# second-state/qwen3_asr_rs

Hardware: AMD Instinct MI355X
Metric: audio-seconds/sec (RTFx) Qwen3-ASR-0.6B greedy, 30s clips (higher is better)
Workload: dtype bf16; 1 GPU; Qwen3-ASR-0.6b bf16, batch=1 x 30s synthetic 16kHz clip per GPU, 100 new tokens (fixed, EOS ignored); clips_per_gpu=1, parallelism=dp1 (independent utterances per GPU, no data-path collective)

## Files before the change

### qwen3_asr_rs_amd/csrc/engine.cpp

```cpp
#include <hip/hip_runtime.h>

#include <sched.h>

#include <chrono>
#include <cmath>
#include <cstdio>
#include <cstring>
#include <map>
#include <memory>
#include <mutex>
#include <thread>

#include "engine_internal.h"

using namespace q3a;

namespace {

thread_local std::string g_last_error;

constexpr int kGemvMaxSeq = 2;

template <typename T>
void upload(DevBuf& b, const std::vector<T>& v, hipStream_t s) {
// ... 416 lines not shown
  }
  void enqueue_beam_round() {
    const int W = beam_w_, S = B, U = B / W;
    BeamTopkArgs t{};
    t.logits = logits.as<float>(); t.S = S; t.V = d.vocab; t.W = W;
    t.cand_val = beam_cand_val.as<float>(); t.cand_idx = beam_cand_idx.as<int>();
    t.part_max = beam_part_max.as<float>(); t.part_sum = beam_part_sum.as<float>();
    t.out_ids = beam_topk_ids.as<int>(); t.out_lp = beam_topk_lp.as<float>();
    timed(Q3A_KC_ARGMAX, 0, [&] { KCHK(launch_beam_topk(t, stream)); });
    BeamAdvanceArgs a{};
    a.U = U; a.W = W; a.topk_ids = t.out_ids; a.topk_lp = t.out_lp;
    a.score = beam_score.as<float>(); a.finished = beam_finished.as<uint8_t>();
    a.parent = beam_parent.as<int>(); a.token = beam_token.as<int>(); a.feed = beam_feed.as<int>();
    a.hist_parent = beam_hist_parent.as<int>(); a.hist_token = beam_hist_token.as<int>(); a.hist_lp = beam_hist_lp.as<float>();
    a.hist_cap = max_new; a.state = beam_state.as<int>();
    a.pos = d_pos.as<int>(); a.lo = beam_lo.as<int>(); a.hi_bias = -1;
    a.host_progress = host_prog_dev + 2; a.eos0 = kEos0; a.eos1 = kEos1;
    timed(Q3A_KC_ARGMAX, 0, [&] { KCHK(launch_beam_advance(a, stream)); });
    KvReorderArgs r{};
    r.kcache = kcache.p; r.vcache = vcache.p; r.elem_bytes = (int)kv_elem(); r.layers = d.dec_layers; r.S = S; r.n_kv = d.n_kv; r.max_ctx = max_ctx;
    r.parent = a.parent; r.lo = a.lo; r.hi = a.pos; r.hi_bias = -1; r.all_done = a.state + BEAM_ST_ALL_DONE;
    timed(Q3A_KC_OTHER, 0, [&] { KCHK(launch_kv_reorder(r, stream)); });
    timed(Q3A_KC_OTHER, 0, [&] { enqueue_set_tokens(a.feed); });
  }
};

enum class Stage { None, Batch, Mel, Encoded, Decoding };

class CallState {
  Stage stage_ = Stage::None;
  int beam_w_ = 0;
  bool fixed_mode_ = false;
  bool head_logits_ = true;
 public:
  bool at(Stage s) const { return stage_ >= s; }
  const int& beam_w() const { return beam_w_; }
  bool fixed_mode() const { return fixed_mode_; }
  const bool& head_logits() const { return head_logits_; }
  void advance(Stage s) { if (stage_ < s) stage_ = s; }
  void rewind(Stage s) {
    if (stage_ > s) stage_ = s;
    if (stage_ < Stage::Decoding) end_search();
  }
  void drop_decode_state() { rewind(Stage::Encoded); }
  void require(Stage s, const char* text) const { if (stage_ < s) fail(text); }
  void require(Stage s, const std::string& text) const { require(s, text.c_str()); }
  void begin_search(int W) { beam_w_ = W; }
  void end_search() { beam_w_ = 0; }
  void begin_call(bool fixed, bool keep_logits) { fixed_mode_ = fixed; head_logits_ = keep_logits; }
  void begin_step_call() { head_logits_ = true; }
};

}

struct q3a_engine : CallState {
  Dims d;
  ArenaLayout L;
  q3a_opts opts{};
  int device = 0;
  hipStream_t stream = nullptr;
  uint8_t* arena = nullptr;
  bool own_arena = false;
  uint32_t arena_flags = 0;
  std::string err;

  DevBuf dft, filt_t, pos_emb;
  int rope_positions = 0;

  int B = 0;
  std::vector<int64_t> n_samples, pcm_off, mel_off;
  std::vector<int> n_frames, n_chunks, T, tok_off;
  int total_chunks = 0, total_T = 0, max_frames = 0;
  std::vector<int> P, seq_off;
  int total_P = 0, max_ctx = 0, max_new = 0;
  std::vector<AttnSeg> enc_segs_h;
  int enc_max_seg = 0;

  DevBuf pcm, d_pcm_off, d_n_samples, d_mel_off, d_n_frames, mel, gmax, d_chunk_utt, d_chunk_frame0;
  DevBuf conv1, conv2, conv3, conv3_rowmap, convout_rowmap;
  DevBuf enc_x, enc_ln, enc_qkv, enc_ctx, enc_ffn, enc_segs, audio_embeds;
  DevBuf ids, audio_rowmap, row_seq, row_pos, dec_segs, last_rows;
  DevBuf dec_x, dec_ln, dec_qkv, dec_ctx, dec_act;
  DevBuf lm_q_buf, lm_qs_buf;
  const int8_t* lm_q = nullptr; const float* lm_qs = nullptr;
  int lm_q_cols = 0;
  DevBuf enc_ctx16, dec_ctx16;
  DevBuf dec_q16;
  int n_cu = 256;
  int* host_prog = nullptr;
  int* host_prog_dev = nullptr;
  DevBuf zero_page;
  int part_stride = 0, attn_nsplit = 0;
  size_t kv_layer_elems = 0;

  int gsize = 32;
  int k_parallel_groups = 1, k_skinny_q = 1, k_dattn_batched_min_wgs = 128, k_skinny_glu_hp3 = 1, k_lm_head_prune = 1;
  std::vector<hipStream_t> chain_streams;
  std::vector<hipEvent_t> join_ev;
  hipEvent_t fork_ev = nullptr;

  static constexpr size_t kGraphCacheMax = 16;
  std::vector<std::pair<std::string, hipGraphExec_t>> graph_cache;
  int pos_hi_ = 0, live_nsplit_ = 0;
  int min_P_ = 0;

  hipStream_t up_stream = nullptr;
  void* pin_p = nullptr;
  size_t pin_cap = 0;
  std::vector<hipEvent_t> up_ev;
  hipEvent_t up_t0 = nullptr, up_t1 = nullptr;
  q3a_io_timings io{};
  bool geom_valid = false;

  q3a_timings timings{};
  hipEvent_t ev[5] = {nullptr, nullptr, nullptr, nullptr, nullptr};
  std::vector<ProfEvent>* prof = nullptr;
  Taps taps;

  bool logit_bias_on_ = false;
  int logit_bias_finite_ = 0;
  bool sampling_on_ = false;
  uint32_t samp_words_[4] = {0, 0, 0, 0};
  bool logit_bias_eos_open_ = true;
  bool repetition_on_ = false;
  float rep_penalty_ = 1.f;
  int rep_ngram_ = 0;

  DecodeStep step{StepView{d, L, opts, arena, arena_flags, stream, chain_streams, join_ev, fork_ev, n_cu, host_prog_dev, prof, taps, lm_q, lm_qs, lm_q_cols,
                           B, max_ctx, max_new, gsize, live_nsplit_, attn_nsplit, min_P_, part_stride, beam_w(), kv_layer_elems, head_logits(),
                           k_parallel_groups, k_skinny_q, k_dattn_batched_min_wgs, k_skinny_glu_hp3, k_lm_head_prune, logit_bias_on_, sampling_on_, repetition_on_}};

  bool precise() const { return step.precise(); }
  bool token_lp() const { return step.token_lp(); }
  bool kv_f32() const { return step.kv_f32(); }
  size_t kv_elem() const { return step.kv_elem(); }
  size_t act_elem() const { return precise() ? 4 : 2; }
  bool valu_attn() const { return precise() || opts.valu_attention; }
  const float* wf(uint64_t off) const { return step.wf(off); }
  const uint16_t* wh(uint64_t off) const { return step.wh(off); }

  void tap(const char* name, const void* ptr, size_t bytes) { step.tap(name, ptr, bytes); }
  void tap_act(const char* name, const void* ptr, size_t elems) {
    if (!opts.debug_taps || elems == 0 || opts.debug_taps == 2) return;
    if (precise()) return tap(name, ptr, elems * 4);
    KCHK(launch_from_bf16((const uint16_t*)ptr, taps.reserve(name, elems * 4).as<float>(), elems, stream));
  }

  void act_gemm(const DevBuf& x, int lda, const uint16_t* W, int M, int N, int K, const GemmEpilogue& ep, bool glu) {
    if (precise()) KCHK(launch_gemm(x.as<float>(), lda, W, M, N, K, ep, glu, true, stream));
    else KCHK(launch_gemm16(x.as<uint16_t>(), lda, W, M, N, K, ep, glu, stream));
// ... 149 lines not shown
    upload(d_n_frames, n_frames, stream);
    upload(d_chunk_utt, chunk_utt, stream);
    upload(d_chunk_frame0, chunk_frame0, stream);
    upload(convout_rowmap, convout_map, stream);
    upload(conv3_rowmap, conv3_map, stream);
    upload(enc_segs, enc_segs_h, stream);
    mel.ensure((size_t)mo * 4);
    gmax.ensure((size_t)b * 4);
    HIPCHK(hipStreamSynchronize(stream));
    B = b;
    geom_valid = true;
    advance(Stage::Batch);
  }

  void upload_pcm(const float* host, const int64_t* ns, int b) {
    set_batch(ns, b);
    int64_t src = 0;
    for (int u = 0; u < b; ++u) {
      HIPCHK(hipMemcpyAsync(pcm.as<float>() + pcm_off[u], host + src, (size_t)ns[u] * 4, hipMemcpyHostToDevice, stream));
      src += ns[u];
    }
    HIPCHK(hipStreamSynchronize(stream));
  }

  void upload_ptrs_and_mel(const float* const* ptrs, const int64_t* ns, int b) {
    const auto w0 = std::chrono::steady_clock::now();
    set_batch(ns, b);
    static const int mode = [] { const char* e = getenv("Q3A_UPLOAD_MODE"); return e ? atoi(e) : 1; }();
    static const int thr_env = [] { const char* e = getenv("Q3A_UPLOAD_THREADS"); return e ? atoi(e) : -1; }();
    static const int pieces_env = [] { const char* e = getenv("Q3A_UPLOAD_PIECES"); return e ? atoi(e) : 8; }();
    io = q3a_io_timings{};
    io.mode = mode;
    HIPCHK(hipEventRecord(ev[0], stream));
    const size_t total = (size_t)(pcm_off[b - 1] + ((ns[b - 1] + 3) & ~int64_t(3))) * 4;
    bool staged = mode != 0;
    if (staged && total > pin_cap) {
      if (up_stream) HIPCHK(hipStreamSynchronize(up_stream));
      if (pin_p) (void)hipHostFree(pin_p);
      pin_p = nullptr; pin_cap = 0;
      const size_t want = (total + (size_t(1) << 20) - 1) & ~((size_t(1) << 20) - 1);
      if (hipHostMalloc(&pin_p, want, hipHostMallocDefault) == hipSuccess && pin_p) pin_cap = want;
      else { (void)hipGetLastError(); pin_p = nullptr; staged = false; io.mode = 0; }
    }
    if (!staged) {
      for (int u = 0; u < b; ++u)
        HIPCHK(hipMemcpyAsync(pcm.as<float>() + pcm_off[u], ptrs[u], (size_t)ns[u] * 4, hipMemcpyHostToDevice, stream));
      HIPCHK(hipStreamSynchronize(stream));
      io.pieces = b;
      run_mel();
      HIPCHK(hipEventRecord(ev[1], stream));
      io.stage_ms = std::chrono::duration<float, std::milli>(std::chrono::steady_clock::now() - w0).count();
      return;
    }
    if (!up_stream) {
      HIPCHK(hipStreamCreateWithFlags(&up_stream, hipStreamNonBlocking));
      HIPCHK(hipEventCreate(&up_t0));
      HIPCHK(hipEventCreate(&up_t1));
    }
    HIPCHK(hipStreamSynchronize(up_stream));
    const int want_pieces = std::max(1, std::min(b, pieces_env));
    std::vector<int> first;
    {
      const size_t per = (total + want_pieces - 1) / want_pieces;
      size_t acc = 0;
      first.push_back(0);
      for (int u = 0; u < b; ++u) {
// ... 12 lines not shown
    io.pieces = np;
    io.threads = nthr;
    std::vector<std::atomic<int>> ready(np);
    for (auto& r : ready) r.store(0, std::memory_order_relaxed);
    std::atomic<int> next{0};
    uint8_t* const pin = (uint8_t*)pin_p;
    auto copy_piece = [&](int p) {
      for (int u = first[p]; u < first[p + 1]; ++u) memcpy(pin + (size_t)pcm_off[u] * 4, ptrs[u], (size_t)ns[u] * 4);
      ready[p].store(1, std::memory_order_release);
    };
    struct Joiner {
      std::vector<std::thread> th;
      ~Joiner() { for (auto& t : th) if (t.joinable()) t.join(); }
    } workers;
    for (int t = 0; t < nthr; ++t)
      workers.th.emplace_back([&] { for (int p; (p = next.fetch_add(1, std::memory_order_relaxed)) < np;) copy_piece(p); });
    MelBatch mb{pcm.as<float>(), d_pcm_off.as<int64_t>(), d_n_samples.as<int64_t>(), d_mel_off.as<int64_t>(),
                d_n_frames.as<int>(), mel.as<float>(), gmax.as<unsigned>()};
    HIPCHK(hipEventRecord(up_t0, up_stream));
    for (int p = 0; p < np; ++p) {
      if (nthr == 0) copy_piece(p);
      for (unsigned spins = 0; !ready[p].load(std::memory_order_acquire);)
        if (++spins > 256) sched_yield();
      const int u0 = first[p], u1 = first[p + 1];
      const size_t o0 = (size_t)pcm_off[u0] * 4, o1 = (size_t)(pcm_off[u1 - 1] + ns[u1 - 1]) * 4;
      HIPCHK(hipMemcpyAsync((uint8_t*)pcm.p + o0, pin + o0, o1 - o0, hipMemcpyHostToDevice, up_stream));
      HIPCHK(hipEventRecord(up_ev[p], up_stream));
      HIPCHK(hipStreamWaitEvent(stream, up_ev[p], 0));
      MelBatch piece = mb;
      piece.pcm_off += u0; piece.n_samples += u0; piece.mel_off += u0; piece.n_frames += u0; piece.gmax_key += u0;
      int mf = 0;
      for (int u = u0; u < u1; ++u) mf = std::max(mf, n_frames[u]);
      KCHK(launch_mel(piece, u1 - u0, mf, dft.as<float>(), filt_t.as<float>(), stream));
    }
    HIPCHK(hipEventRecord(up_t1, up_stream));
    io.stage_ms = std::chrono::duration<float, std::milli>(std::chrono::steady_clock::now() - w0).count();
    mel_done();
    HIPCHK(hipEventRecord(ev[1], stream));
  }

  void run_mel() {
    MelBatch mb{pcm.as<float>(), d_pcm_off.as<int64_t>(), d_n_samples.as<int64_t>(), d_mel_off.as<int64_t>(),
                d_n_frames.as<int>(), mel.as<float>(), gmax.as<unsigned>()};
    KCHK(launch_mel(mb, B, max_frames, dft.as<float>(), filt_t.as<float>(), stream));
    mel_done();
  }
  void mel_done() {
    advance(Stage::Mel);
    size_t bytes = 0;
    for (int u = 0; u < B; ++u) bytes += (size_t)n_frames[u] * d.n_mels * 4;
    tap("mel", mel.p, bytes);
  }

  void run_encoder() {
    require(Stage::Mel, "q3a_encode: no mel (call q3a_mel first)");
    const int C = d.conv_ch, D = d.enc_d, Fn = d.enc_ffn;
    const int H1 = Dims::conv_len(d.n_mels), W1 = Dims::conv_len(d.chunk_frames());
    const int H2 = Dims::conv_len(H1), W2 = Dims::conv_len(W1);
    const int H3 = Dims::conv_len(H2), W3 = Dims::conv_len(W2);
    const bool sp = precise();
    const size_t nch = (size_t)total_chunks;
    const size_t ae = act_elem();
    conv1.ensure(nch * H1 * W1 * C * ae);
    conv2.ensure(nch * H2 * W2 * C * ae);
    conv3.ensure(nch * H3 * W3 * C * ae);
    const size_t Tt = (size_t)total_T;
    const bool qkv16 = !valu_attn();
    enc_x.ensure(Tt * D * 4); enc_ln.ensure(Tt * D * ae); enc_qkv.ensure(Tt * 3 * D * (qkv16 ? 2 : 4));
    enc_ctx.ensure(Tt * D * (valu_attn() ? 4 : ae));
    if (valu_attn() && !sp) enc_ctx16.ensure(Tt * D * 2);
    enc_ffn.ensure(Tt * Fn * ae); audio_embeds.ensure(Tt * d.enc_out * 4);

    ChunkTable ct{d_chunk_utt.as<int>(), d_chunk_frame0.as<int>()};
    KCHK(launch_conv1(mel.as<float>(), d_mel_off.as<int64_t>(), d_n_frames.as<int>(), ct, total_chunks, d.n_mels,
                      d.chunk_frames(), wf(L.conv1_w), wf(L.conv1_b), C, conv1.as<float>(), stream, act16(conv1)));
    tap_act("conv1", conv1.p, nch * H1 * W1 * C);
    {
// ... 50 lines not shown
      KCHK(launch_layernorm(enc_x.as<float>(), wf(e.ln2_w), wf(e.ln2_b), enc_ln.as<float>(), total_T, D, 1e-5f, stream, act16(enc_ln)));
      {
        GemmEpilogue ep; act_out(ep, enc_ffn); ep.ldo = Fn; ep.bias = wf(e.fc1_b); ep.act = 1;
        act_gemm(enc_ln, D, wh(e.fc1_w), total_T, Fn, D, ep, false);
      }
      {
        GemmEpilogue ep; ep.out = enc_x.as<float>(); ep.ldo = D; ep.bias = wf(e.fc2_b); ep.resid = enc_x.as<float>();
        act_gemm(enc_ffn, Fn, wh(e.fc2_w), total_T, D, Fn, ep, false);
      }
      if (li == 0) tap("enc_layer0", enc_x.p, Tt * D * 4);
      if (opts.debug_taps == 1 && knobs().layer_taps.load() != 0) {
        char name[32];
        snprintf(name, sizeof(name), "E%02d_x", li);
        tap(name, enc_x.p, Tt * D * 4);
      }
    }
    tap("enc_last", enc_x.p, Tt * D * 4);
    KCHK(launch_layernorm(enc_x.as<float>(), wf(L.ln_post_w), wf(L.ln_post_b), enc_ln.as<float>(), total_T, D, 1e-5f, stream, act16(enc_ln)));
    {
      GemmEpilogue ep; act_out(ep, enc_ffn); ep.ldo = D; ep.bias = wf(L.proj1_b); ep.act = 1;
      act_gemm(enc_ln, D, wh(L.proj1_w), total_T, D, D, ep, false);
    }
    {
      GemmEpilogue ep; ep.out = audio_embeds.as<float>(); ep.ldo = d.enc_out; ep.bias = wf(L.proj2_b);
      act_gemm(enc_ffn, D, wh(L.proj2_w), total_T, d.enc_out, D, ep, false);
    }
    tap("audio_embeds", audio_embeds.p, Tt * d.enc_out * 4);
    HIPCHK(hipGetLastError());
    advance(Stage::Encoded);
  }

  void setup_prompts(const int32_t* ids_h, const int32_t* lens, int b, int max_new_req, bool before_encoder = false) {
    if (!before_encoder) require_encoded("q3a_prefill", b);
    P.assign(lens, lens + b);
    end_search();
    seq_off.resize(b);
    std::vector<int> rowseq, rowpos, amap((size_t)total_T, -1), last(b);
    int off = 0, maxP = 0;
    for (int s = 0; s < b; ++s) {
      seq_off[s] = off;
      int na = 0;
      for (int i = 0; i < P[s]; ++i) {
        rowseq.push_back(s);
        rowpos.push_back(i);
        int id = ids_h[off + i];
        if (id < 0 || id >= d.vocab) fail("q3a_prefill: token id out of range");
        if (id == kAudioPad) {
          if (na >= T[s]) fail("q3a_prefill: more <|audio_pad|> tokens than encoder tokens");
          amap[(size_t)tok_off[s] + na] = off + i;
          ++na;
        }
      }
      if (na != T[s]) fail("q3a_prefill: number of <|audio_pad|> tokens does not match the encoder output length");
      if (P[s] <= 0) fail("q3a_prefill: empty prompt");
      last[s] = off + P[s] - 1;
      off += P[s];
      maxP = std::max(maxP, P[s]);
    }
    total_P = off;
    max_new = std::min(std::max(max_new_req, 1), opts.max_new_tokens);
    max_ctx = ((maxP + max_new + 1 + 127) / 128) * 128;
    pos_hi_ = maxP;
    min_P_ = *std::min_element(P.begin(), P.end());
    {
      static const int pad = [] { const char* e = getenv("Q3A_CTX_PAD"); return e ? atoi(e) : 0; }();
      if (pad > 0) max_ctx += (pad + 127) / 128 * 128;
    }
    ensure_rope(max_ctx + 1);
    std::vector<int> ids_v(ids_h, ids_h + total_P);
    std::vector<AttnSeg> segs(b);
    for (int s = 0; s < b; ++s)
      segs[s] = AttnSeg{seq_off[s], P[s], (int64_t)s * d.n_kv * max_ctx * 128};
    upload(ids, ids_v, stream);
    upload(row_seq, rowseq, stream);
    upload(row_pos, rowpos, stream);
    upload(audio_rowmap, amap, stream);
    upload(last_rows, last, stream);
    upload(dec_segs, segs, stream);
    upload(step.d_pos, P, stream);
    const size_t Pt = (size_t)total_P, H = d.hidden;
    dec_x.ensure(Pt * H * 4); dec_ln.ensure(Pt * H * act_elem()); dec_qkv.ensure(Pt * d.qkv_dim() * 4);
    dec_ctx.ensure(Pt * d.q_dim() * (valu_attn() ? 4 : act_elem())); dec_act.ensure(Pt * d.inter * act_elem());
    if (!valu_attn()) dec_q16.ensure(Pt * d.q_dim() * 2);
    if (valu_attn() && !precise()) dec_ctx16.ensure(Pt * d.q_dim() * 2);
    kv_layer_elems = (size_t)b * d.n_kv * max_ctx * 128;
    step.kcache.ensure(kv_layer_elems * d.dec_layers * kv_elem());
    step.vcache.ensure(kv_layer_elems * d.dec_layers * kv_elem());
    step.rope_cur.ensure((size_t)b * 128 * 4);
    {
      Knobs& kn = knobs();
      const int gs = kn.decode_group_size.load();
      gsize = (gs >= 1 && gs <= 32) ? gs : 32;
      k_parallel_groups = kn.decode_parallel_groups.load(); k_skinny_q = kn.skinny_q.load();
      k_dattn_batched_min_wgs = kn.dattn_batched_min_wgs.load();
      k_skinny_glu_hp3 = kn.skinny_glu_hp3.load();
      k_lm_head_prune = kn.lm_head_prune.load();
    }
    const size_t ng = (size_t)step.n_groups(b);
    step.nn_x.ensure(ng * 32 * H * 2); step.nn_ss.ensure((size_t)ng * (H / 8) * 32 * 4);
    step.x_dec.ensure((size_t)b * H * 4); step.next_tok.ensure((size_t)b * 4); step.forced_tok.ensure((size_t)b * 4); step.draft_accepted.ensure((size_t)b * 8);
    step.out_ids.ensure((size_t)b * max_new * 4); step.step_count.ensure((size_t)b * 4); step.done.ensure((size_t)b);
    step.s_ln.ensure((size_t)b * H * 4); step.s_qkv.ensure((size_t)b * d.qkv_dim() * 4); step.s_ctx.ensure(ng * 32 * d.q_dim() * 4);
    step.s_act.ensure(ng * 32 * d.inter * 4); step.logits.ensure((size_t)b * d.vocab * 4);
    part_stride = std::max(128, (d.vocab + 3) / 4);
    step.part_val.ensure((size_t)b * part_stride * 4); step.part_idx.ensure((size_t)b * part_stride * 4);
    if (token_lp()) { step.part_sum.ensure((size_t)b * part_stride * 4); step.out_lp.ensure((size_t)b * max_new * 4); }
    if (sampling_on_) { step.samp_max.ensure((size_t)b * sample_chunks(d.vocab) * 4); step.samp_sum.ensure((size_t)b * sample_chunks(d.vocab) * 4); }
    {
      const size_t nblk4 = ((size_t)(d.vocab + 15) / 16 + 3) & ~size_t(3);
      step.blk_lo.ensure(nblk4 * 4); step.blk_hi.ensure(nblk4 * 4);
    }
    attn_nsplit = (max_ctx + dattn_keys_per_split(kv_f32()) - 1) / dattn_keys_per_split(kv_f32());
    {
      const size_t n_stat = (size_t)b * d.n_q * attn_nsplit;
      step.attn_pm.ensure((n_stat + 8) * 4); step.attn_pl.ensure((n_stat + 8) * 4);
      step.attn_po.ensure(n_stat * 128 * 4);
      if (knobs().poison_attn_partials.load() != 0) {
        HIPCHK(hipMemsetAsync(step.attn_pm.p, 0xFF, step.attn_pm.cap, stream));
        HIPCHK(hipMemsetAsync(step.attn_pl.p, 0xFF, step.attn_pl.cap, stream));
        HIPCHK(hipMemsetAsync(step.attn_po.p, 0xFF, step.attn_po.cap, stream));
      }
    }
    HIPCHK(hipMemsetAsync(step.step_count.p, 0, (size_t)b * 4, stream));
    HIPCHK(hipMemsetAsync(step.done.p, 0, (size_t)b, stream));
    HIPCHK(hipMemsetAsync(step.n_done.p, 0, 64, stream));
    HIPCHK(hipMemsetAsync(step.out_ids.p, 0, (size_t)b * max_new * 4, stream));
    if (token_lp()) HIPCHK(hipMemsetAsync(step.out_lp.p, 0, (size_t)b * max_new * 4, stream));
    HIPCHK(hipStreamSynchronize(stream));
    for (auto cs : chain_streams) HIPCHK(hipStreamSynchronize(cs));
    __atomic_store_n(&host_prog[0], 0, __ATOMIC_RELAXED);
    __atomic_store_n(&host_prog[1], 0, __ATOMIC_RELAXED);
    drain_retired_graphs();
    {
      bool any = false;
      DecodeStep::each_buf(step, [&](DevBuf& sb) { any = any || sb.grew; sb.grew = false; });
      if (any) drop_graphs();
    }
  }

  void run_prefill() {
    run_prefill_layers();
    const int H = d.hidden;
    KCHK(launch_gather_rows(dec_x.as<float>(), last_rows.as<int>(), B, H, step.x_dec.as<float>(), stream));
    tap("dec_last_hidden", step.x_dec.p, (size_t)B * H * 4);
    step.run_head(0);
    tap("logits", step.logits.p, (size_t)B * d.vocab * 4);
    HIPCHK(hipGetLastError());
    advance(Stage::Decoding);
  }

  void run_prefill_layers() {
    drop_decode_state();
    const int H = d.hidden, I = d.inter, QD = d.q_dim(), QKV = d.qkv_dim();
    const bool sp = precise();
    KCHK(launch_embed(ids.as<int>(), total_P, wh(L.embed), H, kAudioPad, dec_x.as<float>(), stream));
    KCHK(launch_scatter_rows(audio_embeds.as<float>(), audio_rowmap.as<int>(), total_T, d.hidden, dec_x.as<float>(), stream));
    tap("dec_embed", dec_x.p, (size_t)total_P * H * 4);
    AttnArgs at{};
    at.q = dec_qkv.as<float>(); at.q_rs = QKV; at.kv_hs = (int64_t)max_ctx * 128; at.kv_rs = 128;
    at.o = dec_ctx.as<float>(); at.o_rs = QD; at.segs = dec_segs.as<AttnSeg>(); at.n_segs = B;
    at.max_len = *std::max_element(P.begin(), P.end()); at.n_kv_heads = d.n_kv;
    at.scale_div = sqrtf((float)d.head_dim);
    at.o16 = valu_attn() ? nullptr : dec_ctx.as<uint16_t>();
    if (!valu_attn()) { at.q16 = dec_q16.as<uint16_t>(); at.q_rs = QD; }
    const DevBuf& ctx_in = (valu_attn() && !sp) ? dec_ctx16 : dec_ctx;
    auto proj_gemm = [&](const DevBuf& x, const DecodeStep::Proj& p, GemmEpilogue ep) {
      ep.bias = p.bias;
      act_gemm(x, p.K, p.W, total_P, p.N, p.K, ep, p.mode == 2);
    };
    const bool fuse_rope = knobs().fuse_qkrope.load() != 0 && !valu_attn() && !precise() && d.head_dim == 128 && gemm256_eligible(total_P, QKV, H) && H % 64 == 0;
// ... 301 lines not shown
    return exec;
  }
  hipGraphExec_t graph_for_step() {
    const std::string sig = make_graph_sig();
    for (size_t i = 0; i < graph_cache.size(); ++i)
      if (graph_cache[i].first == sig) {
        if (i + 1 != graph_cache.size()) std::rotate(graph_cache.begin() + i, graph_cache.begin() + i + 1, graph_cache.end());
        return graph_cache.back().second;
      }
    const hipGraphExec_t exec = capture_graph([&] { enqueue_step(); });
    ++graph_captures_;
    if (graph_cache.size() >= kGraphCacheMax) {
      retired_graphs.push_back(graph_cache.front().second);
      graph_cache.erase(graph_cache.begin());
    }
    graph_cache.emplace_back(sig, exec);
    return exec;
  }
  std::vector<hipGraphExec_t> retired_graphs;
  int32_t graph_captures_ = 0;
  void drain_retired_graphs() {
    for (auto ge : retired_graphs) (void)hipGraphExecDestroy(ge);
    retired_graphs.clear();
  }
  void drop_graphs() {
    drain_retired_graphs();
    for (auto& ge : graph_cache) (void)hipGraphExecDestroy(ge.second);
    graph_cache.clear();
  }

  void decode_steps(int n) {
    require(Stage::Decoding, "decode: no prefill state");
    if (n <= 0) return;
    const bool eager = !opts.use_graph || prof;
    const int kps = dattn_keys_per_split(kv_f32());
    for (int i = 0; i < n; ++i) {
      live_nsplit_ = step.uses_key_splits() ? std::min(attn_nsplit, pos_hi_ / kps + 1) : attn_nsplit;
      if (eager) enqueue_step();
      else HIPCHK(hipGraphLaunch(graph_for_step(), stream));
      ++pos_hi_;
    }
    if (eager) HIPCHK(hipGetLastError());
  }

  int max_new_request(int max_new_req, int fixed_new) const { return fixed_new > 0 ? fixed_new : max_new_req > 0 ? max_new_req : opts.max_new_tokens; }
  std::pair<std::vector<int32_t>, std::vector<int32_t>> asr_prompts(const int32_t* lang_ids, int n_prefix) const {
    return concat_prompts(B, [&](int s, int32_t* dst) {
      int32_t len = 0;
      q3a_build_prompt(T[s], lang_ids, n_prefix, dst, &len);
      return len;
    });
  }

  template <class Prompts>
  void whole_path_front(const char* what, const float* const* pcm16k, const int64_t* ns_in, int n, int width, int max_new_req, Prompts&& prompts) {
    if (!pcm16k || !ns_in || n < 1) fail(std::string(what) + ": bad argument");
    require_utterance_ptrs(what, pcm16k, n);
    HIPCHK(hipSetDevice(device));
    const int b = n * width;
    std::vector<const float*> ptrs((size_t)b);
    std::vector<int64_t> ns((size_t)b);
    for (int s = 0; s < b; ++s) { ptrs[s] = pcm16k[s / width]; ns[s] = ns_in[s / width]; }
    set_batch(ns.data(), b);
    auto&& [ids_v, lens_v] = prompts();
    setup_prompts(ids_v.data(), lens_v.data(), b, max_new_req, true);
    timings = q3a_timings{};
    upload_ptrs_and_mel(ptrs.data(), ns.data(), b);
    run_encoder();
  }

  void run_resident(int fixed_new, bool front_done = false) {
    if (!front_done) {
      HIPCHK(hipEventRecord(ev[0], stream));
      run_mel();
      HIPCHK(hipEventRecord(ev[1], stream));
      run_encoder();
    }
    HIPCHK(hipEventRecord(ev[2], stream));
    run_prefill();
    HIPCHK(hipEventRecord(ev[3], stream));
    int steps = 0;
    static const bool host_timing = [] { const char* e = getenv("Q3A_DEBUG_HOST_TIMING"); return e && atoi(e) != 0; }();
    const auto h0 = std::chrono::steady_clock::now();
    if (fixed_new > 0) {
      steps = fixed_new - 1;
      decode_steps(steps);
      if (host_timing) fprintf(stderr, "[q3a host timing] %d graph launches enqueued in %.1f us\n", steps,
                               std::chrono::duration<double, std::micro>(std::chrono::steady_clock::now() - h0).count());
    } else {
      steps = run_ahead(host_prog, max_new - 1, "greedy");
    }
    HIPCHK(hipEventRecord(ev[4], stream));
    HIPCHK(hipStreamSynchronize(stream));
    HIPCHK(hipGetLastError());
    decode_timings(steps);
  }

  void fetch_ids(int32_t* out, int stride, int32_t* out_lens) {
    if (!at(Stage::Decoding) || beam_w() > 0) fail("q3a_fetch_ids: nothing generated");
    fetch_generated<int32_t>(nullptr, out, stride, out_lens);
  }
  void fetch_logprobs(float* out, int stride, int32_t* out_lens) {
    if (!token_lp()) fail("q3a_fetch_logprobs: the engine was created without opts.token_logprobs = 1");
    require(Stage::Decoding, "q3a_fetch_logprobs: nothing generated");
    fetch_generated<float>(&step.out_lp, out, stride, out_lens);
  }
  template <class T> void fetch_generated(const DevBuf* vals, T* out, int stride, int32_t* out_lens) {
    std::vector<int> ids((size_t)B * max_new);
    std::vector<T> v(vals ? ids.size() : 0);
    HIPCHK(hipMemcpy(ids.data(), step.out_ids.p, ids.size() * 4, hipMemcpyDeviceToHost));
    if (vals) HIPCHK(hipMemcpy(v.data(), vals->p, v.size() * sizeof(T), hipMemcpyDeviceToHost));
    generated_lens(ids, out_lens);
    for (int s = 0; s < B; ++s)
      for (int i = 0; i < std::min(out_lens[s], stride); ++i) out[(size_t)s * stride + i] = vals ? v[(size_t)s * max_new + i] : (T)ids[(size_t)s * max_new + i];
  }
  void generated_lens(const std::vector<int>& all, int32_t* out_lens) {
    std::vector<int> sc(B);
    HIPCHK(hipMemcpy(sc.data(), step.step_count.p, (size_t)B * 4, hipMemcpyDeviceToHost));
    for (int s = 0; s < B; ++s) {
      int n = std::min(sc[s], max_new), len = 0;
      for (; len < n; ++len) {
        int t = all[(size_t)s * max_new + len];
        if (!fixed_mode() && (t == kEos0 || t == kEos1)) break;
      }
      out_lens[s] = len;
    }
  }

  int beam_dbg_S_ = 0, beam_dbg_W_ = 0;
  int* beam_prog() const { return host_prog + 2; }

  void beam_check(const char* what, int W) const {
    if (W < 1 || W > BEAM_MAX_W) fail(std::string(what) + ": width must be 1..8");
    if (B % W != 0) fail(std::string(what) + ": the batch of " + std::to_string(B) + " sequences is not divisible by width " + std::to_string(W));
    if (B > 32) fail(std::string(what) + ": utterances x width = " + std::to_string(B) + " exceeds 32 sequences");
    for (int s = 0; s < B; ++s)
      if (P[s] != P[s / W * W]) fail(std::string(what) + ": the prompts of utterance " + std::to_string(s / W) + " differ in length (its " + std::to_string(W) + " slots must hold the same prompt)");
    if (d.vocab < W) fail(std::string(what) + ": vocabulary smaller than the width");
  }
  void set_logit_bias(const int32_t* ids, const float* bias, int n, float default_bias) {
    const char* what = "q3a_set_logit_bias";
    require_asr(what);
    const int V = d.vocab;
    if (n < 0 || (n > 0 && (!ids || !bias))) fail(std::string(what) + ": bad argument");
    if (!(default_bias == 0.f || default_bias == -INFINITY)) fail(std::string(what) + ": default_bias must be 0 or -inf");
    std::vector<float> b((size_t)V, default_bias);
    std::vector<uint8_t> seen((size_t)V, 0);
    for (int i = 0; i < n; ++i) {
      const int id = ids[i];
      if (id < 0 || id >= V) fail(std::string(what) + ": id " + std::to_string(id) + " is outside the vocabulary (" + std::to_string(V) + ")");
      if (seen[id]) fail(std::string(what) + ": duplicate id " + std::to_string(id));
// ... 139 lines not shown
      std::stable_sort(order.begin(), order.end(), [&](int x, int y) { return sc[u * W + x] > sc[u * W + y]; });
      for (int k = 0; k < W; ++k) {
        const int q = u * W + order[k];
        toks.clear(); lps.clear();
        for (int r = R - 1, cur = q; r >= 0; --r) {
          const size_t h = (size_t)r * S + cur;
          if (ht[h] >= 0) { toks.push_back(ht[h]); lps.push_back(hl[h]); }
          cur = hp[h];
        }
        std::reverse(toks.begin(), toks.end());
        std::reverse(lps.begin(), lps.end());
        const int n_lp = (int)toks.size();
        if (fin[q] && !toks.empty()) toks.pop_back();
        const int n = (int)toks.size();
        if (n > stride) fail("q3a_beam_fetch: a hypothesis has " + std::to_string(n) + " ids, more than stride " + std::to_string(stride));
        const size_t o = (size_t)u * W + k;
        for (int i = 0; i < n; ++i) out[o * stride + i] = toks[i];
        out_lens[o] = n;
        if (out_scores) out_scores[o] = sc[q];
        if (out_fin) out_fin[o] = fin[q];
        if (out_lp)
          for (int i = 0; i < n_lp && i < stride + 1; ++i) out_lp[o * (stride + 1) + i] = lps[i];
      }
    }
  }

  ~q3a_engine() {
    drop_graphs();
    for (auto cs : chain_streams) (void)hipStreamDestroy(cs);
    for (auto ce : join_ev) (void)hipEventDestroy(ce);
    if (fork_ev) (void)hipEventDestroy(fork_ev);
    if (own_arena && arena) (void)hipFree(arena);
    if (host_prog) (void)hipHostFree(host_prog);
    if (up_stream) { (void)hipStreamSynchronize(up_stream); (void)hipStreamDestroy(up_stream); }
    if (pin_p) (void)hipHostFree(pin_p);
    for (auto ue : up_ev) (void)hipEventDestroy(ue);
    if (up_t0) (void)hipEventDestroy(up_t0);
    if (up_t1) (void)hipEventDestroy(up_t1);
    for (auto& x : ev)
      if (x) (void)hipEventDestroy(x);
    if (stream) (void)hipStreamDestroy(stream);
  }
};


namespace q3a {
void set_thread_error(const std::string& msg) { g_last_error = msg; }
void set_error(q3a_engine* e, const char* msg) {
  if (e) e->err = msg;
  g_last_error = msg;
}
}

extern "C" {

void q3a_opts_default(q3a_opts* o) {
  memset(o, 0, sizeof(*o));
  o->precise = 0;
  o->max_new_tokens = 4096;
  o->use_graph = 1;
  o->debug_taps = 0;
}

static int32_t create_impl(const char* model_dir, int32_t device, void* dev_arena, uint64_t bytes, const q3a_opts* opts,
                           q3a_engine** out) {
  q3a_engine* e = nullptr;
// ... 331 lines not shown
  if (next_ids) HIPCHK(hipMemcpy(next_ids, e->step.next_tok.p, (size_t)B * 4, hipMemcpyDeviceToHost));
  Q3A_CATCH(e)
}

int32_t q3a_decode_step(q3a_engine* e, int32_t* next_ids, uint8_t* done, float* logits_out) {
  if (!e) return 1;
  Q3A_TRY(e)
  e->require_asr("q3a_decode_step");
  if (e->beam_w() > 0) fail("q3a_decode_step: a beam search owns the decode state (q3a_beam_step; a new q3a_prefill returns to the greedy step)");
  HIPCHK(hipSetDevice(e->device));
  {
    std::vector<int> pos(e->B);
    HIPCHK(hipMemcpy(pos.data(), e->step.d_pos.p, (size_t)e->B * 4, hipMemcpyDeviceToHost));
    for (int s = 0; s < e->B; ++s)
      if (pos[s] + 1 > e->max_ctx) fail("q3a_decode_step: KV cache capacity exhausted (max_new_tokens reached)");
  }
  e->begin_step_call();
  e->decode_steps(1);
  HIPCHK(hipStreamSynchronize(e->stream));
  HIPCHK(hipGetLastError());
  if (next_ids) HIPCHK(hipMemcpy(next_ids, e->step.next_tok.p, (size_t)e->B * 4, hipMemcpyDeviceToHost));
  if (done) HIPCHK(hipMemcpy(done, e->step.done.p, (size_t)e->B, hipMemcpyDeviceToHost));
  if (logits_out) HIPCHK(hipMemcpy(logits_out, e->step.logits.p, (size_t)e->B * e->d.vocab * 4, hipMemcpyDeviceToHost));
  Q3A_CATCH(e)
}

int32_t q3a_set_next_tokens(q3a_engine* e, const int32_t* ids, int32_t B) {
  if (!e) return 1;
  Q3A_TRY(e)
  HIPCHK(hipSetDevice(e->device));
  if (!e->at(Stage::Decoding) || B != e->B || e->beam_w() > 0) fail("q3a_set_next_tokens: no decode state / batch mismatch");
  for (int s = 0; s < B; ++s)
    if (ids[s] < 0 || ids[s] >= e->d.vocab) fail("q3a_set_next_tokens: token id out of range");
  e->step.enqueue_forced_tokens(ids);
  HIPCHK(hipStreamSynchronize(e->stream));
  Q3A_CATCH(e)
}

int32_t q3a_run_resident(q3a_engine* e, const int32_t* lang_prefix_ids, int32_t n_prefix, int32_t max_new,
                         int32_t fixed_new_tokens) {
  if (!e) return 1;
  Q3A_TRY(e)
  e->require_asr("q3a_run_resident");
  HIPCHK(hipSetDevice(e->device));
  e->begin_call(fixed_new_tokens > 0, e->opts.debug_taps != 0);
  e->rewind(Stage::Batch);
  e->require(Stage::Batch, "q3a_run_resident: no batch uploaded");
  const auto pr = e->asr_prompts(lang_prefix_ids, n_prefix);
  e->setup_prompts(pr.first.data(), pr.second.data(), e->B, e->max_new_request(max_new, fixed_new_tokens), true);
  e->run_resident(fixed_new_tokens);
  Q3A_CATCH(e)
}

int32_t q3a_fetch_ids(q3a_engine* e, int32_t* out_ids, int32_t stride, int32_t* out_lens) {
  if (!e) return 1;
  Q3A_TRY(e)
  HIPCHK(hipSetDevice(e->device));
  e->fetch_ids(out_ids, stride, out_lens);
  Q3A_CATCH(e)
}

int32_t q3a_fetch_logprobs(q3a_engine* e, float* out_lp, int32_t stride, int32_t* out_lens) {
  if (!e) return 1;
  Q3A_TRY(e)
  if (!out_lens || (stride > 0 && !out_lp)) fail("q3a_fetch_logprobs: bad argument");
  HIPCHK(hipSetDevice(e->device));
  e->fetch_logprobs(out_lp, stride, out_lens);
  Q3A_CATCH(e)
}

int32_t q3a_transcribe_batch_ptrs(q3a_engine* e, const float* const* pcm16k, const int64_t* n_samples, int32_t B,
                                  const int32_t* lang_prefix_ids, int32_t n_prefix, int32_t max_new, int32_t fixed_new_tokens,
                                  int32_t* out_ids, int32_t stride, int32_t* out_lens) {
  if (!e) return 1;
  Q3A_TRY(e)
  e->require_asr("q3a_transcribe_batch");
// ... 70 lines not shown
  std::vector<int> acc;
  std::vector<int32_t> cur, cur_lens(B), nxt;
  {
    size_t total = 0;
    for (int s = 0; s < B; ++s) { cur_lens[s] = draft_lens[s]; total += draft_lens[s]; }
    if (total) cur.assign(draft_ids, draft_ids + total);
  }
  for (int round = 0;; ++round) {
    e->run_prefill_draft(dp, acc, nullptr);
    int tail = 0;
    for (int s = 0; s < B; ++s) tail = std::max(tail, cur_lens[s] - acc[s] - 1);
    if (round + 1 >= max_rounds || tail < std::max(min_tail, 1)) break;
    nxt.clear();
    size_t off = 0;
    for (int s = 0; s < B; ++s) {
      int32_t need = 0;
      const size_t o = nxt.size();
      nxt.resize(o + (size_t)cur_lens[s] + 1);
      if (q3a_draft_next_round(cur.data() + off, cur_lens[s], acc[s], acc[(size_t)B + s], nxt.data() + o, cur_lens[s] + 1, &need) != 0)
        fail(std::string(what) + ": " + q3a_last_error(nullptr));
      off += cur_lens[s];
      cur_lens[s] = std::min(need, mn_eff);
      nxt.resize(o + cur_lens[s]);
    }
    cur.swap(nxt);
    dp = e->given_plan(what, q3a_engine::kDrafted, pr.first.data(), pr.second.data(), cur.data(), cur_lens.data(), B, mn_eff);
    e->setup_prompts(dp.ids.data(), dp.lens.data(), B, mn);
  }
  HIPCHK(hipEventRecord(e->ev[3], e->stream));
  int min_k = e->max_new;
  for (int s = 0; s < B; ++s) min_k = std::min(min_k, acc[s]);
  const int steps = e->run_ahead(e->host_prog, e->max_new - 1 - min_k, "draft", acc[0]);
  HIPCHK(hipEventRecord(e->ev[4], e->stream));
  HIPCHK(hipStreamSynchronize(e->stream));
  HIPCHK(hipGetLastError());
  e->decode_timings(steps);
  e->fetch_ids(out_ids, stride, out_lens);
  if (accepted_out)
    for (int s = 0; s < B; ++s) accepted_out[s] = acc[s];
  e->io.wall_ms = std::chrono::duration<float, std::milli>(std::chrono::steady_clock::now() - w0).count();
  Q3A_CATCH(e)
}

int32_t q3a_io_timings_last(const q3a_engine* e, q3a_io_timings* out) {
  if (!e || !out) return 1;
  *out = e->io;
  return 0;
}

int32_t q3a_stage_timings(const q3a_engine* e, q3a_timings* out) {
  if (!e || !out) return 1;
  *out = e->timings;
  return 0;
}

int32_t q3a_profile_decode_step(q3a_engine* e, q3a_kernel_profile* out) {
  if (!e || !out) return 1;
  Q3A_TRY(e)
  HIPCHK(hipSetDevice(e->device));
  e->require(Stage::Decoding, "q3a_profile_decode_step: no decode state");
  std::vector<ProfEvent> evs;
  e->prof = &evs;
  try {
    e->decode_steps(1);
    HIPCHK(hipStreamSynchronize(e->stream));
  } catch (...) {
    e->prof = nullptr;
// ... 144 lines not shown
```

### qwen3_asr_rs_amd/csrc/engine_internal.h

```cpp
#pragma once
#include <hip/hip_runtime.h>

#include <algorithm>
#include <atomic>
#include <cstdint>
#include <string>
#include <vector>

#include "../../include/q3asr.h"
#include "kernels.h"
#include "model.h"

#define HIPCHK(expr) q3a::hip_check((expr), __FILE__, __LINE__, #expr)
#define KCHK(expr) q3a::kernel_check(expr)

namespace q3a {

inline void hip_check(hipError_t e, const char* file, int line, const char* expr) {
  if (e != hipSuccess) fail(std::string("HIP error: ") + hipGetErrorString(e) + " at " + file + ":" + std::to_string(line) + " (" + expr + ")");
}
inline void kernel_check(const char* msg) { if (msg) fail(std::string("kernel launch: ") + msg); }

constexpr int kAudioPad = 151676, kEos0 = 151643, kEos1 = 151645;

inline std::atomic<uint64_t> g_device_bytes{0};

struct DevBuf {
  void* p = nullptr;
  size_t cap = 0;
  bool grew = false;
  DevBuf() = default;
  DevBuf(DevBuf&& o) noexcept { *this = std::move(o); }
  DevBuf& operator=(DevBuf&& o) noexcept { std::swap(p, o.p); std::swap(cap, o.cap); std::swap(grew, o.grew); return *this; }
  ~DevBuf() { release(); }
  void ensure(size_t bytes) {
    if (bytes <= cap) return;
    release();
    size_t want = (bytes + 255) & ~size_t(255);
    HIPCHK(hipMalloc(&p, want));
    cap = want;
    g_device_bytes += want;
    grew = true;
  }
  void release() {
    if (p) { (void)hipFree(p); g_device_bytes -= cap; }
    p = nullptr;
    cap = 0;
  }
  template <typename T> T* as() const { return reinterpret_cast<T*>(p); }
};

void set_error(q3a_engine* e, const char* msg);

}

#define Q3A_TRY(e) try {
#define Q3A_CATCH(e)                                                                  \
  }                                                                                   \
  catch (const std::exception& ex) { q3a::set_error(e, ex.what()); return 1; }        \
  catch (...) { q3a::set_error(e, "unknown error"); return 1; }                       \
  return 0;
```

Before: 499.0 audio-seconds/sec.

## Batch prompt table uploads into one pinned copy and prefetch results asynchronously

Prompt tables (ids, row maps, segments, positions) are now built directly in a pinned staging buffer and sent with one async copy into a single device allocation, replacing seven separate uploads. The blocking stream syncs at the end of setup are gone, and idle streams are only synced when they are busy. Generated ids and step counts are copied to pinned host memory before the final sync so fetch_ids can read them without further blocking copies. Debug host-timing stamps are also added. This trims per-call host latency but adds state-tracking (publish/retract) that must stay consistent across all API paths.

```diff
diff --git a/qwen3_asr_rs_amd/csrc/engine.cpp b/qwen3_asr_rs_amd/csrc/engine.cpp
--- a/qwen3_asr_rs_amd/csrc/engine.cpp
+++ b/qwen3_asr_rs_amd/csrc/engine.cpp
@@ -472,6 +472,7 @@
   int beam_w_ = 0;
   bool fixed_mode_ = false;
   bool head_logits_ = true;
+  bool results_on_host_ = false;
  public:
   bool at(Stage s) const { return stage_ >= s; }
   const int& beam_w() const { return beam_w_; }
@@ -480,15 +481,18 @@
   void advance(Stage s) { if (stage_ < s) stage_ = s; }
   void rewind(Stage s) {
     if (stage_ > s) stage_ = s;
-    if (stage_ < Stage::Decoding) end_search();
+    if (stage_ < Stage::Decoding) { end_search(); retract_results(); }
   }
   void drop_decode_state() { rewind(Stage::Encoded); }
   void require(Stage s, const char* text) const { if (stage_ < s) fail(text); }
   void require(Stage s, const std::string& text) const { require(s, text.c_str()); }
-  void begin_search(int W) { beam_w_ = W; }
+  void begin_search(int W) { beam_w_ = W; retract_results(); }
   void end_search() { beam_w_ = 0; }
-  void begin_call(bool fixed, bool keep_logits) { fixed_mode_ = fixed; head_logits_ = keep_logits; }
-  void begin_step_call() { head_logits_ = true; }
+  void begin_call(bool fixed, bool keep_logits) { fixed_mode_ = fixed; head_logits_ = keep_logits; retract_results(); }
+  void begin_step_call() { head_logits_ = true; retract_results(); }
+  bool results_on_host() const { return results_on_host_ && stage_ == Stage::Decoding; }
+  void publish_results() { results_on_host_ = stage_ == Stage::Decoding; }
+  void retract_results() { results_on_host_ = false; }
 };
 
 }
@@ -519,7 +523,10 @@
   DevBuf pcm, d_pcm_off, d_n_samples, d_mel_off, d_n_frames, mel, gmax, d_chunk_utt, d_chunk_frame0;
   DevBuf conv1, conv2, conv3, conv3_rowmap, convout_rowmap;
   DevBuf enc_x, enc_ln, enc_qkv, enc_ctx, enc_ffn, enc_segs, audio_embeds;
-  DevBuf ids, audio_rowmap, row_seq, row_pos, dec_segs, last_rows;
+  DevSpan ids, audio_rowmap, row_seq, row_pos, dec_segs, last_rows;
+  DevBuf prompt_tabs;
+  PinnedBuf prompt_stage;
+  PinnedBuf result_host;
   DevBuf dec_x, dec_ln, dec_qkv, dec_ctx, dec_act;
   DevBuf lm_q_buf, lm_qs_buf;
   const int8_t* lm_q = nullptr; const float* lm_qs = nullptr;
@@ -556,6 +563,16 @@
   hipEvent_t ev[5] = {nullptr, nullptr, nullptr, nullptr, nullptr};
   std::vector<ProfEvent>* prof = nullptr;
   Taps taps;
+  using HostClock = std::chrono::steady_clock;
+  struct HostStamps { HostClock::time_point entry, drained, tables, uploaded, first_kernel, ev0, ev4; bool armed = false; } stamps;
+  static bool host_timing() {
+    static const bool on = [] { const char* e = getenv("Q3A_DEBUG_HOST_TIMING"); return e && atoi(e) != 0; }();
+    return on;
+  }
+  static double us_between(HostClock::time_point a, HostClock::time_point b) { return std::chrono::duration<double, std::micro>(b - a).count(); }
+  void stamp_entry() { if (host_timing()) { stamps.entry = HostClock::now(); stamps.armed = true; } }
+  void stamp_first_kernel() { if (stamps.armed) { stamps.first_kernel = HostClock::now(); stamps.armed = false; } }
+  void stamp(HostClock::time_point HostStamps::*which) { if (host_timing()) stamps.*which = HostClock::now(); }
 
   bool logit_bias_on_ = false;
   int logit_bias_finite_ = 0;
@@ -771,6 +788,7 @@
     io = q3a_io_timings{};
     io.mode = mode;
     HIPCHK(hipEventRecord(ev[0], stream));
+    stamp(&HostStamps::ev0);
     const size_t total = (size_t)(pcm_off[b - 1] + ((ns[b - 1] + 3) & ~int64_t(3))) * 4;
     bool staged = mode != 0;
     if (staged && total > pin_cap) {
@@ -849,6 +867,7 @@
       int mf = 0;
       for (int u = u0; u < u1; ++u) mf = std::max(mf, n_frames[u]);
       KCHK(launch_mel(piece, u1 - u0, mf, dft.as<float>(), filt_t.as<float>(), stream));
+      stamp_first_kernel();
     }
     HIPCHK(hipEventRecord(up_t1, up_stream));
     io.stage_ms = std::chrono::duration<float, std::milli>(std::chrono::steady_clock::now() - w0).count();
@@ -860,6 +879,7 @@
     MelBatch mb{pcm.as<float>(), d_pcm_off.as<int64_t>(), d_n_samples.as<int64_t>(), d_mel_off.as<int64_t>(),
                 d_n_frames.as<int>(), mel.as<float>(), gmax.as<unsigned>()};
     KCHK(launch_mel(mb, B, max_frames, dft.as<float>(), filt_t.as<float>(), stream));
+    stamp_first_kernel();
     mel_done();
   }
   void mel_done() {
@@ -976,17 +996,29 @@
 
   void setup_prompts(const int32_t* ids_h, const int32_t* lens, int b, int max_new_req, bool before_encoder = false) {
     if (!before_encoder) require_encoded("q3a_prefill", b);
+    drain_for_call();
+    stamp(&HostStamps::drained);
     P.assign(lens, lens + b);
     end_search();
     seq_off.resize(b);
-    std::vector<int> rowseq, rowpos, amap((size_t)total_T, -1), last(b);
+    size_t n_rows = 0;
+    for (int s = 0; s < b; ++s) n_rows += (size_t)std::max(P[s], 0);
+    const auto up256 = [](size_t x) { return (x + 255) & ~size_t(255); };
+    const size_t o_ids = 0, o_rowseq = o_ids + up256(n_rows * 4), o_rowpos = o_rowseq + up256(n_rows * 4), o_amap = o_rowpos + up256(n_rows * 4),
+                 o_last = o_amap + up256((size_t)total_T * 4), o_segs = o_last + up256((size_t)b * 4), o_pos = o_segs + up256((size_t)b * sizeof(AttnSeg)),
+                 o_end = o_pos + up256((size_t)b * 4);
+    prompt_stage.ensure(o_end);
+    uint8_t* const st = prompt_stage.as<uint8_t>();
+    int32_t* const ids_st = (int32_t*)(st + o_ids);
+    int *const rowseq = (int*)(st + o_rowseq), *const rowpos = (int*)(st + o_rowpos), *const amap = (int*)(st + o_amap), *const last = (int*)(st + o_last);
+    std::fill(amap, amap + total_T, -1);
     int off = 0, maxP = 0;
     for (int s = 0; s < b; ++s) {
       seq_off[s] = off;
       int na = 0;
       for (int i = 0; i < P[s]; ++i) {
-        rowseq.push_back(s);
-        rowpos.push_back(i);
+        rowseq[off + i] = s;
+        rowpos[off + i] = i;
         int id = ids_h[off + i];
         if (id < 0 || id >= d.vocab) fail("q3a_prefill: token id out of range");
         if (id == kAudioPad) {
@@ -994,6 +1026,7 @@
           amap[(size_t)tok_off[s] + na] = off + i;
           ++na;
         }
+        ids_st[off + i] = id;
       }
       if (na != T[s]) fail("q3a_prefill: number of <|audio_pad|> tokens does not match the encoder output length");
       if (P[s] <= 0) fail("q3a_prefill: empty prompt");
@@ -1011,17 +1044,17 @@
       if (pad > 0) max_ctx += (pad + 127) / 128 * 128;
     }
     ensure_rope(max_ctx + 1);
-    std::vector<int> ids_v(ids_h, ids_h + total_P);
-    std::vector<AttnSeg> segs(b);
-    for (int s = 0; s < b; ++s)
-      segs[s] = AttnSeg{seq_off[s], P[s], (int64_t)s * d.n_kv * max_ctx * 128};
-    upload(ids, ids_v, stream);
-    upload(row_seq, rowseq, stream);
-    upload(row_pos, rowpos, stream);
-    upload(audio_rowmap, amap, stream);
-    upload(last_rows, last, stream);
-    upload(dec_segs, segs, stream);
-    upload(step.d_pos, P, stream);
+    for (int s = 0; s < b; ++s) {
+      ((AttnSeg*)(st + o_segs))[s] = AttnSeg{seq_off[s], P[s], (int64_t)s * d.n_kv * max_ctx * 128};
+      ((int*)(st + o_pos))[s] = P[s];
+    }
+    prompt_tabs.ensure(o_pos);
+    {
+      uint8_t* const dv = prompt_tabs.as<uint8_t>();
+      ids.p = dv + o_ids; row_seq.p = dv + o_rowseq; row_pos.p = dv + o_rowpos; audio_rowmap.p = dv + o_amap; last_rows.p = dv + o_last; dec_segs.p = dv + o_segs;
+    }
+    step.d_pos.ensure(std::max<size_t>((size_t)b * 4, 16));
+    result_host.ensure(result_off(b, max_new, 3));
     const size_t Pt = (size_t)total_P, H = d.hidden;
     dec_x.ensure(Pt * H * 4); dec_ln.ensure(Pt * H * act_elem()); dec_qkv.ensure(Pt * d.qkv_dim() * 4);
     dec_ctx.ensure(Pt * d.q_dim() * (valu_attn() ? 4 : act_elem())); dec_act.ensure(Pt * d.inter * act_elem());
@@ -1059,27 +1092,50 @@
       const size_t n_stat = (size_t)b * d.n_q * attn_nsplit;
       step.attn_pm.ensure((n_stat + 8) * 4); step.attn_pl.ensure((n_stat + 8) * 4);
       step.attn_po.ensure(n_stat * 128 * 4);
-      if (knobs().poison_attn_partials.load() != 0) {
-        HIPCHK(hipMemsetAsync(step.attn_pm.p, 0xFF, step.attn_pm.cap, stream));
-        HIPCHK(hipMemsetAsync(step.attn_pl.p, 0xFF, step.attn_pl.cap, stream));
-        HIPCHK(hipMemsetAsync(step.attn_po.p, 0xFF, step.attn_po.cap, stream));
-      }
+    }
+    {
+      bool any = false;
+      DecodeStep::each_buf(step, [&](DevBuf& sb) { any = any || sb.grew; sb.grew = false; });
+      if (any) drop_graphs();
+    }
+    stamp(&HostStamps::tables);
+    HIPCHK(hipMemcpyAsync(prompt_tabs.p, st, o_pos, hipMemcpyHostToDevice, stream));
+    HIPCHK(hipMemcpyAsync(step.d_pos.p, st + o_pos, (size_t)b * 4, hipMemcpyHostToDevice, stream));
+    if (knobs().poison_attn_partials.load() != 0) {
+      HIPCHK(hipMemsetAsync(step.attn_pm.p, 0xFF, step.attn_pm.cap, stream));
+      HIPCHK(hipMemsetAsync(step.attn_pl.p, 0xFF, step.attn_pl.cap, stream));
+      HIPCHK(hipMemsetAsync(step.attn_po.p, 0xFF, step.attn_po.cap, stream));
     }
     HIPCHK(hipMemsetAsync(step.step_count.p, 0, (size_t)b * 4, stream));
     HIPCHK(hipMemsetAsync(step.done.p, 0, (size_t)b, stream));
     HIPCHK(hipMemsetAsync(step.n_done.p, 0, 64, stream));
     HIPCHK(hipMemsetAsync(step.out_ids.p, 0, (size_t)b * max_new * 4, stream));
     if (token_lp()) HIPCHK(hipMemsetAsync(step.out_lp.p, 0, (size_t)b * max_new * 4, stream));
-    HIPCHK(hipStreamSynchronize(stream));
-    for (auto cs : chain_streams) HIPCHK(hipStreamSynchronize(cs));
+    stamp(&HostStamps::uploaded);
+  }
+  void drain_for_call() {
+    const auto idle = [](hipStream_t s) {
+      if (hipStreamQuery(s) == hipSuccess) return;
+      (void)hipGetLastError();
+      HIPCHK(hipStreamSynchronize(s));
+    };
+    idle(stream);
+    for (auto cs : chain_streams) idle(cs);
     __atomic_store_n(&host_prog[0], 0, __ATOMIC_RELAXED);
     __atomic_store_n(&host_prog[1], 0, __ATOMIC_RELAXED);
     drain_retired_graphs();
-    {
-      bool any = false;
-      DecodeStep::each_buf(step, [&](DevBuf& sb) { any = any || sb.grew; sb.grew = false; });
-      if (any) drop_graphs();
-    }
+    retract_results();
+  }
+  static size_t result_off(int b, int mn, int k) {
+    const size_t ids = (((size_t)b * mn * 4) + 255) & ~size_t(255), cnt = (((size_t)b * 4) + 255) & ~size_t(255);
+    return k == 0 ? 0 : k == 1 ? ids : k == 2 ? ids + cnt : 2 * ids + cnt;
+  }
+  void enqueue_result_copy() {
+    uint8_t* const h = result_host.as<uint8_t>();
+    const size_t n = (size_t)B * max_new * 4;
+    HIPCHK(hipMemcpyAsync(h + result_off(B, max_new, 0), step.out_ids.p, n, hipMemcpyDeviceToHost, stream));
+    HIPCHK(hipMemcpyAsync(h + result_off(B, max_new, 1), step.step_count.p, (size_t)B * 4, hipMemcpyDeviceToHost, stream));
+    if (token_lp()) HIPCHK(hipMemcpyAsync(h + result_off(B, max_new, 2), step.out_lp.p, n, hipMemcpyDeviceToHost, stream));
   }
 
   void run_prefill() {
@@ -1447,6 +1503,7 @@
   void decode_steps(int n) {
     require(Stage::Decoding, "decode: no prefill state");
     if (n <= 0) return;
+    retract_results();
     const bool eager = !opts.use_graph || prof;
     const int kps = dattn_keys_per_split(kv_f32());
     for (int i = 0; i < n; ++i) {
@@ -1469,6 +1526,7 @@
 
   template <class Prompts>
   void whole_path_front(const char* what, const float* const* pcm16k, const int64_t* ns_in, int n, int width, int max_new_req, Prompts&& prompts) {
+    stamp_entry();
     if (!pcm16k || !ns_in || n < 1) fail(std::string(what) + ": bad argument");
     require_utterance_ptrs(what, pcm16k, n);
     HIPCHK(hipSetDevice(device));
@@ -1487,6 +1545,7 @@
   void run_resident(int fixed_new, bool front_done = false) {
     if (!front_done) {
       HIPCHK(hipEventRecord(ev[0], stream));
+      stamp(&HostStamps::ev0);
       run_mel();
       HIPCHK(hipEventRecord(ev[1], stream));
       run_encoder();
@@ -1495,25 +1554,34 @@
     run_prefill();
     HIPCHK(hipEventRecord(ev[3], stream));
     int steps = 0;
-    static const bool host_timing = [] { const char* e = getenv("Q3A_DEBUG_HOST_TIMING"); return e && atoi(e) != 0; }();
     const auto h0 = std::chrono::steady_clock::now();
     if (fixed_new > 0) {
       steps = fixed_new - 1;
       decode_steps(steps);
-      if (host_timing) fprintf(stderr, "[q3a host timing] %d graph launches enqueued in %.1f us\n", steps,
+      if (host_timing()) fprintf(stderr, "[q3a host timing] %d graph launches enqueued in %.1f us\n", steps,
                                std::chrono::duration<double, std::micro>(std::chrono::steady_clock::now() - h0).count());
     } else {
       steps = run_ahead(host_prog, max_new - 1, "greedy");
     }
     HIPCHK(hipEventRecord(ev[4], stream));
+    stamp(&HostStamps::ev4);
+    enqueue_result_copy();
     HIPCHK(hipStreamSynchronize(stream));
+    publish_results();
+    if (host_timing())
+      fprintf(stderr, "[q3a host timing] call ends: entry -> first kernel enqueued %.1f us, entry -> ev[0] recorded %.1f us, ev[4] recorded -> synchronised %.1f us; "
+              "prompts: entry -> drained %.1f us, tables and buffers %.1f us, copy and fills enqueued %.1f us\n",
+              us_between(stamps.entry, stamps.first_kernel), us_between(stamps.entry, stamps.ev0), us_between(stamps.ev4, HostClock::now()),
+              us_between(stamps.entry, stamps.drained), us_between(stamps.drained, stamps.tables), us_between(stamps.tables, stamps.uploaded));
     HIPCHK(hipGetLastError());
     decode_timings(steps);
   }
 
   void fetch_ids(int32_t* out, int stride, int32_t* out_lens) {
     if (!at(Stage::Decoding) || beam_w() > 0) fail("q3a_fetch_ids: nothing generated");
+    const auto f0 = HostClock::now();
     fetch_generated<int32_t>(nullptr, out, stride, out_lens);
+    if (host_timing()) fprintf(stderr, "[q3a host timing] fetch_ids %.1f us\n", us_between(f0, HostClock::now()));
   }
   void fetch_logprobs(float* out, int stride, int32_t* out_lens) {
     if (!token_lp()) fail("q3a_fetch_logprobs: the engine was created without opts.token_logprobs = 1");
@@ -1521,17 +1589,27 @@
     fetch_generated<float>(&step.out_lp, out, stride, out_lens);
   }
   template <class T> void fetch_generated(const DevBuf* vals, T* out, int stride, int32_t* out_lens) {
-    std::vector<int> ids((size_t)B * max_new);
-    std::vector<T> v(vals ? ids.size() : 0);
-    HIPCHK(hipMemcpy(ids.data(), step.out_ids.p, ids.size() * 4, hipMemcpyDeviceToHost));
-    if (vals) HIPCHK(hipMemcpy(v.data(), vals->p, v.size() * sizeof(T), hipMemcpyDeviceToHost));
-    generated_lens(ids, out_lens);
+    const size_t n = (size_t)B * max_new;
+    std::vector<int> ids_v, sc_v;
+    std::vector<T> v_v;
+    const int *ids = nullptr, *sc = nullptr;
+    const T* v = nullptr;
+    if (results_on_host()) {
+      const uint8_t* const h = result_host.as<uint8_t>();
+      ids = (const int*)(h + result_off(B, max_new, 0)); sc = (const int*)(h + result_off(B, max_new, 1));
+      if (vals) v = (const T*)(h + result_off(B, max_new, 2));
+    } else {
+      ids_v.resize(n); sc_v.resize(B); v_v.resize(vals ? n : 0);
+      HIPCHK(hipMemcpy(ids_v.data(), step.out_ids.p, n * 4, hipMemcpyDeviceToHost));
+      if (vals) HIPCHK(hipMemcpy(v_v.data(), vals->p, n * sizeof(T), hipMemcpyDeviceToHost));
+      HIPCHK(hipMemcpy(sc_v.data(), step.step_count.p, (size_t)B * 4, hipMemcpyDeviceToHost));
+      ids = ids_v.data(); sc = sc_v.data(); v = v_v.data();
+    }
+    generated_lens(ids, sc, out_lens);
     for (int s = 0; s < B; ++s)
       for (int i = 0; i < std::min(out_lens[s], stride); ++i) out[(size_t)s * stride + i] = vals ? v[(size_t)s * max_new + i] : (T)ids[(size_t)s * max_new + i];
   }
-  void generated_lens(const std::vector<int>& all, int32_t* out_lens) {
-    std::vector<int> sc(B);
-    HIPCHK(hipMemcpy(sc.data(), step.step_count.p, (size_t)B * 4, hipMemcpyDeviceToHost));
+  void generated_lens(const int* all, const int* sc, int32_t* out_lens) {
     for (int s = 0; s < B; ++s) {
       int n = std::min(sc[s], max_new), len = 0;
       for (; len < n; ++len) {
@@ -1737,6 +1815,7 @@
     if (fork_ev) (void)hipEventDestroy(fork_ev);
     if (own_arena && arena) (void)hipFree(arena);
     if (host_prog) (void)hipHostFree(host_prog);
+    prompt_stage.release(); result_host.release();
     if (up_stream) { (void)hipStreamSynchronize(up_stream); (void)hipStreamDestroy(up_stream); }
     if (pin_p) (void)hipHostFree(pin_p);
     for (auto ue : up_ev) (void)hipEventDestroy(ue);
@@ -2134,6 +2213,7 @@
   if (!e->at(Stage::Decoding) || B != e->B || e->beam_w() > 0) fail("q3a_set_next_tokens: no decode state / batch mismatch");
   for (int s = 0; s < B; ++s)
     if (ids[s] < 0 || ids[s] >= e->d.vocab) fail("q3a_set_next_tokens: token id out of range");
+  e->retract_results();
   e->step.enqueue_forced_tokens(ids);
   HIPCHK(hipStreamSynchronize(e->stream));
   Q3A_CATCH(e)
@@ -2144,6 +2224,7 @@
   if (!e) return 1;
   Q3A_TRY(e)
   e->require_asr("q3a_run_resident");
+  e->stamp_entry();
   HIPCHK(hipSetDevice(e->device));
   e->begin_call(fixed_new_tokens > 0, e->opts.debug_taps != 0);
   e->rewind(Stage::Batch);
@@ -2280,7 +2361,9 @@
   for (int s = 0; s < B; ++s) min_k = std::min(min_k, acc[s]);
   const int steps = e->run_ahead(e->host_prog, e->max_new - 1 - min_k, "draft", acc[0]);
   HIPCHK(hipEventRecord(e->ev[4], e->stream));
+  e->enqueue_result_copy();
   HIPCHK(hipStreamSynchronize(e->stream));
+  e->publish_results();
   HIPCHK(hipGetLastError());
   e->decode_timings(steps);
   e->fetch_ids(out_ids, stride, out_lens);
diff --git a/qwen3_asr_rs_amd/csrc/engine_internal.h b/qwen3_asr_rs_amd/csrc/engine_internal.h
--- a/qwen3_asr_rs_amd/csrc/engine_internal.h
+++ b/qwen3_asr_rs_amd/csrc/engine_internal.h
@@ -50,6 +50,33 @@
   template <typename T> T* as() const { return reinterpret_cast<T*>(p); }
 };
 
+struct DevSpan {
+  void* p = nullptr;
+  template <typename T> T* as() const { return reinterpret_cast<T*>(p); }
+};
+
+struct PinnedBuf {
+  void* p = nullptr;
+  size_t cap = 0;
+  PinnedBuf() = default;
+  PinnedBuf(const PinnedBuf&) = delete;
+  PinnedBuf& operator=(const PinnedBuf&) = delete;
+  ~PinnedBuf() { release(); }
+  void ensure(size_t bytes) {
+    if (bytes <= cap) return;
+    release();
+    size_t want = (bytes + 4095) & ~size_t(4095);
+    HIPCHK(hipHostMalloc(&p, want, hipHostMallocDefault));
+    cap = want;
+  }
+  void release() {
+    if (p) (void)hipHostFree(p);
+    p = nullptr;
+    cap = 0;
+  }
+  template <typename T> T* as() const { return reinterpret_cast<T*>(p); }
+};
+
 void set_error(q3a_engine* e, const char* msg);
 
 }
```

Measured after the change: 497.7 audio-seconds/sec, median of 2. Within noise of the previous version (-0.3%).
